# xtcyclist/hash_join_codes_KNL

Measured on AMD Instinct MI355X. Metric: probe Gtuples/s + % HBM roofline, PHJ |R|=64M join |S|=1G, 1/2/4/8 GPU, higher is better.
Workload: dtype u32

## Files before the change

### hash_join_codes_knl_amd/build.py

```python
import os
import shutil
import subprocess
import sys

PKG = os.path.dirname(os.path.abspath(__file__))
ROOT = os.path.dirname(PKG)
CSRC = os.path.join(PKG, "csrc")
HOST = os.path.join(PKG, "host")
LIB = os.path.join(PKG, "lib")
ARCH = "gfx950"

KERNEL_SOURCES = ["partition_kernels.hip", "join_kernels.hip", "npj_kernels.hip",
                  "gen_kernels.hip", "audit_kernels.hip", "hjgpu_api.hip", "hjgpu_ops.hip", "hjgpu_colops.hip", "hjgpu_host.hip", "hjgpu_multi.hip"]
HOST_PROGRAMS = {"npj": "npj_main.cpp", "phj": "phj_main.cpp", "cpra": "cpra_main.cpp",
                 "write": "write_main.cpp"}


def _hipcc():
    for cand in (os.environ.get("HIPCC"), shutil.which("hipcc"), "/opt/rocm/bin/hipcc"):
        if cand and os.path.exists(cand):
            return cand
    raise RuntimeError("hipcc not found (ROCm toolchain required to build libhjgpu)")


KERNEL_HASH_FILES = ["partition_kernels.hip", "join_kernels.hip", "npj_kernels.hip", "hj_device.hpp",
                     "hj_emit.hpp", "hj_lookup.hpp", "hj_internal.hpp", "scatter_layout.hpp", "hjgpu_ctx.hpp", "hjgpu_api.hip", "hjgpu_ops.hip",
                     "hjgpu_colops.hip", "colop_checks.hpp"]


def kernel_hash():
    import hashlib
    h = hashlib.sha256()
    for f in KERNEL_HASH_FILES:
        with open(os.path.join(CSRC, f), "rb") as fh:
            h.update(fh.read())
    return h.hexdigest()[:16]


def library_hash():
    import hashlib
    h = hashlib.sha256()
    for f in sorted(os.listdir(CSRC)):
        if f.endswith((".hip", ".hpp")):
            h.update(f.encode())
            with open(os.path.join(CSRC, f), "rb") as fh:
                h.update(fh.read())
    with open(os.path.join(ROOT, "include", "hjgpu.h"), "rb") as fh:
        h.update(fh.read())
    return h.hexdigest()[:16]


def _newer(target, deps):
    if not os.path.exists(target):
        return True
    t = os.path.getmtime(target)
    return any(os.path.getmtime(d) > t for d in deps if os.path.exists(d))


def lib_path():
# ... 65 lines not shown
```

### hash_join_codes_knl_amd/csrc/hjgpu_api.hip

```cpp
#include "hjgpu_ctx.hpp"
#include "hj_device.hpp"

using namespace hjapi;



namespace hjapi {


int fail(hjgpu_ctx *ctx, int status, const char *what, hipError_t e)
{
    if (ctx) {
        if (e != hipSuccess)
            snprintf(ctx->err, sizeof(ctx->err), "%s: %s", what, hipGetErrorString(e));
        else
            snprintf(ctx->err, sizeof(ctx->err), "%s", what);
    }
    return status;
}

static int release(hjgpu_ctx *ctx, void *p)
{
    if (!p) return HJGPU_OK;
    HIPCHK(ctx, hipFree(p));
// ... 189 lines not shown
    uint32_t f1 = prm ? prm->fanout1 : 0, f2 = prm ? prm->fanout2 : 0;
    *big_tables = false;
    if (f1 == 0) {
        double target = tune.join.cap() * 0.85;
        double parts = ceil((double)inner / target);
        if (parts > HJGPU_MAX_PARTS) {
            *big_tables = true;
            target = hj_join_config_big().cap() * 0.85;
            parts = ceil((double)inner / target);
        }
        if (parts < 64) parts = 64;
        if (parts > HJGPU_MAX_PARTS) parts = HJGPU_MAX_PARTS;
        if (parts <= 640) { f1 = (uint32_t)parts; f2 = 1; }
        else {
            f1 = 2;
            while ((double)f1 * f1 * 2.0 < parts) f1 <<= 1;
            if (f1 > 256) f1 = 256;
            if (parts >= 192.0 * 64.0) f1 = 192;
            f2 = (uint32_t)ceil(parts / f1);
            while (f2 > HJGPU_MAX_FANOUT) { f1 <<= 1; f2 = (uint32_t)ceil(parts / f1); }
            while ((u64)f1 * f2 > HJGPU_MAX_PARTS) --f2;
        }
    } else if (f2 == 0) f2 = 1;
    *F1 = f1; *F2 = f2;
}

void record(hjgpu_ctx *ctx, int which, hipStream_t s)
{
    if (ctx->ev_cur) {
        if (which == EV_BEGIN || which == EV_S_HIST || which == EV_S_PLAN || which == EV_S_SC1 || which == EV_S_SC2 || which == EV_JOIN)
            (void)hipEventRecord(ctx->ev_cur[which], s);
        return;
    }
    if (which == EV_BEGIN) { ctx->stats_override = false; ctx->grp_ev_groups = 0; ctx->last_lookup = false; }
    ctx->ev_valid[which] = (hipEventRecord(ctx->ev[which], s) == hipSuccess);
}

int audit_begin(hjgpu_ctx *ctx, int kind, size_t inner, size_t outer, hipStream_t stream, u64 **rec)
{
    *rec = nullptr;
    if (!ctx->tune.audit) return HJGPU_OK;
    const size_t words = (size_t)HJ_AUDIT_STAGES * 4;
    CHK(ensure(ctx, ctx->audit, (size_t)HJ_AUDIT_RING * words * sizeof(u64)));
    u64 *r = reinterpret_cast<u64 *>(ctx->audit.p) + (size_t)(ctx->audit_seq % HJ_AUDIT_RING) * words;
    HIPCHK(ctx, hj_zero_async(r, words * sizeof(u64), stream));
    CHK(hj_audit_meta(r + 4 * (HJ_AUDIT_STAGES - 1), ctx->audit_seq, (u64)kind, (u64)inner, (u64)outer, stream));
    ctx->audit_seq += 1;
    ctx->audit_checks.clear();
    *rec = r;
    return HJGPU_OK;
}

int audit_partitions(hjgpu_ctx *ctx, int stage, const u64 *tuples, const u64 *beg, const u64 *end, uint32_t parts, const HjAuditHash &h, u64 *rec,
                     hipStream_t stream)
{
    ctx->audit_checks.push_back(hjgpu_ctx::AuditCheck{stage, tuples, beg, end, parts, h});
    return hj_audit_partitions(tuples, beg, end, parts, h, rec + 4 * stage, ctx->cus, stream);
}

int refuse_capture(hjgpu_ctx *ctx, hipStream_t stream)
{
    hipStreamCaptureStatus status = hipStreamCaptureStatusNone;
    if (hipStreamIsCapturing(stream, &status) != hipSuccess) { (void)hipGetLastError(); return HJGPU_OK; }
    if (status != hipStreamCaptureStatusNone)
        return fail(ctx, HJGPU_EINVAL, "the stream is capturing a HIP graph: hjgpu joins cannot be captured");
    return HJGPU_OK;
}
// ... 283 lines not shown
    if (pl->F2 > 1 && pl->C == 1 && !ctx->tune.dense2 && ctx->tune.batch_tuples > 0 && pl->F1 <= 1024) {
        const u64 target = (u64)ctx->tune.batch_tuples;
        const u64 tile = gs.tile;
        const u64 tiles = hj_tiles_of(0, outer, 0, (uint32_t)tile) + 1;
        const u64 k = (tiles + ranges_of(ctx->tune, tiles, pl->F1) - 1) / ranges_of(ctx->tune, tiles, pl->F1) + 1;
        const u64 rpb = std::max<u64>(1, target / (k * tile));
        const u64 nb = (gs.ranges_per_chunk + rpb - 1) / rpb + 1;
        if (outer >= 3 * target) {
            pl->batch_ranges = (uint32_t)rpb; pl->batch_cap = (uint32_t)nb; pl->batch_tile_cap = (uint32_t)k;
            const u64 bound = rpb * k * tile;
            pl->tdesc_b_cap = (size_t)(bound / (u64)hj_scatter_tile(ctx->tune, 2, pl->F2, true) + 2 * (u64)pl->F1 + 8);
            pl->batch_bytes = (size_t)(bound + 64) * sizeof(u64);
            CHK(ensure(ctx, ctx->tmp[1], pl->batch_bytes));
            CHK(ensure(ctx, ctx->tmp[3], pl->batch_bytes));
        }
    }
    if (hj_mode_marks_build(pl->mode)) CHK(ensure(ctx, ctx->build_bits, build_bits_bytes(*pl, inner)));
    MetaLayout sz = carve(nullptr, pl->C, pl->F1, pl->P, pl->ranges, pl->items_extra, pl->tiles2, pl->batch_cap, pl->tdesc_b_cap);
    CHK(ensure(ctx, ctx->meta, sz.total_bytes));
    CHK(ensure(ctx, ctx->state, sizeof(DevState)));
    return HJGPU_OK;
}

namespace {

const int EV_OF_S[4] = {EV_S_HIST, EV_S_PLAN, EV_S_SC1, EV_S_SC2};
const int EV_OF_R[4] = {EV_R_HIST, EV_R_PLAN, EV_R_SC1, EV_R_SC2};

struct PhjRoad {
    bool pad2;
    bool merged;
    bool claim;
    bool joins;
};

PhjRoad phj_road(const hjgpu_ctx *ctx, const PhjPlan &pl, const Rel &R, const Rel &S, const EnqueueOpts &o)
{
    PhjRoad w;
    const bool audited = ctx->tune.audit && !o.grp;
    w.pad2 = pl.F2 > 1 && !ctx->tune.dense2;
    const bool resident = o.stages == PHJ_WHOLE && !o.inner_ready && !o.pre;
    w.merged = o.grp || (resident && !pl.batch_ranges && ctx->tune.merged_plan);
    w.claim = w.merged && !o.grp && pl.claim_s && !audited && pl.C == 1 && w.pad2;
    w.joins = R.rows && (S.rows || hj_mode_build_alone(pl.mode)) && o.stages != PHJ_BUILD_ONLY;
    return w;
}

struct PhjRun {
    hjgpu_ctx *ctx;
    const PhjPlan &pl;
    const EnqueueOpts &o;
    const PhjRoad road;
    hipStream_t stream;
    MetaLayout m;
    DevState *st;
    Pass1Geom geom[2];
    const uint32_t *in_k[2], *in_v[2];
    size_t nn[2];
    uint32_t *t1[4], *t2[4];
    PlanArgs pa;
    const u64 *dyn[2];
    u64 *audit = nullptr;
    bool p_major = false;
    uint32_t batches_used = 0;

    PhjRun(hjgpu_ctx *c, const PhjPlan &p, const Rel &R, const Rel &S, const EnqueueOpts &opts, hipStream_t s)
        : ctx(c), pl(p), o(opts), road(phj_road(c, p, R, S, opts)), stream(s),
          m(carve(c->meta.p, p.C, p.F1, p.P, p.ranges, p.items_extra, p.tiles2, p.batch_cap, p.tdesc_b_cap)),
          st(reinterpret_cast<DevState *>(c->state.p)),
          geom{make_geom(c->tune, R.keys, R.rows, p.C, p.F1, true), make_geom(c->tune, S.keys, S.rows, p.C, p.F1, true)},
          in_k{R.keys, S.keys}, in_v{R.vals, S.vals}, nn{R.rows, S.rows},
          t1{(uint32_t *)c->tmp[0].p, nullptr, (uint32_t *)c->tmp[2].p, nullptr},
          t2{(uint32_t *)c->tmp[4].p, nullptr, (uint32_t *)c->tmp[6].p, nullptr},
          dyn{opts.grp ? opts.grp->desc : nullptr, opts.grp ? opts.grp->desc + 2 : nullptr} {}

    bool pieces(int r) const { return o.pre && o.pre->tuples[r]; }

    int setup()
    {
        for (int r = 0; r < 2; ++r) {
            if (pieces(r)) geom[r].align = 0;
            if (!o.pre && (size_t)geom[r].ranges_per_chunk * pl.C > pl.ranges)
                return fail(ctx, HJGPU_EINVAL, "internal: the relation needs more pass-1 ranges than the plan's tables hold");
        }
        pa = plan_args(ctx, m, pl.C, pl.F1, pl.F2, (uint32_t)hj_scatter_tile(ctx->tune, 1, pl.F1, true),
                       (uint32_t)hj_scatter_tile(ctx->tune, 2, pl.F2, true), pl.unique, 0u);
        pa.cap = (uint32_t)hj_join_config_of(ctx->tune, pl.big_tables).cap();
        pa.tdesc_cap = (uint32_t)m.tdesc_cap;
        pa.multi_fill = m.tickets + HJ_TICKET_MULTI_FILL;
        pa.anti = hj_mode_keeps_unmatched(pl.mode) ? 1u : 0u;
        pa.pad2 = road.pad2 ? 1u : 0u;
        p_major = pl.C > 1 && road.pad2 && !o.pre;
        pa.p_major = p_major ? 1u : 0u;
        pa.seg_interleave = (o.pre && pl.C > 1 && road.pad2 && ctx->tune.piece_interleave) ? 1u : 0u;
        if (road.claim) pa.s_cap2 = pl.cap2;
        for (int r = 0; r < 2; ++r) {
            pa.tdesc[r] = m.tdesc[r]; pa.seg2[r] = m.seg2[r]; pa.more[r] = m.more[r]; pa.dyn[r] = dyn[r];
            pa.n[r] = pieces(r) ? o.pre->ch[r].b[pl.C] : nn[r];
            pa.regular[r] = pieces(r) ? 0u : 1u; pa.chunk_part[r] = geom[r].part;
            for (uint32_t c = 0; c < 9; ++c) pa.chunk_beg[r][c] = pieces(r) ? o.pre->ch[r].b[c <= pl.C ? c : pl.C] : geom[r].beg(c);
            pa.in_align[r] = o.pre ? 0u : align_of(in_k[r]);
        }
        return HJGPU_OK;
    }

    int begin()
    {
// ... 8 lines not shown
            HIPCHK(ctx, hj_zero_async(zt, (size_t)(ze - zt), stream));
        }
        if (o.stages == PHJ_PROBE_ONLY) HIPCHK(ctx, hj_zero_async(z1, (size_t)(ze - z1), stream));
        if (o.stages != PHJ_BUILD_ONLY && !o.grp) HIPCHK(ctx, hj_zero_async(st, sizeof(DevState), stream));
        return HJGPU_OK;
    }

    int audit_input(int r)
    {
        if (!audit || !nn[r]) return HJGPU_OK;
        u64 *rec = audit + 4 * (r ? 0 : 3);
        if (o.pre) return o.pre->tuples[r] ? hj_audit_sums_packed(o.pre->tuples[r], o.pre->ch[r].b[0], o.pre->ch[r].b[pl.C], rec, ctx->cus, stream) : HJGPU_OK;
        return in_k[r] ? hj_audit_sums_columns(in_k[r], in_v[r], nn[r], rec, ctx->cus, stream) : HJGPU_OK;
    }
    int audit_pass1(int r)
    {
        if (!audit || !nn[r] || o.pre || pl.C != 1 || pl.F2 <= 1) return HJGPU_OK;
        const HjAuditHash h = {pl.f1, pl.F1, 0u, 1u, 1u, pl.F1};
        return audit_partitions(ctx, r ? 1 : 4, reinterpret_cast<const u64 *>(ctx->tmp[2 * r].p), m.off1[r], nullptr, pl.F1, h, audit, stream);
    }
    int audit_final(int r)
    {
        if (!audit || !nn[r]) return HJGPU_OK;
        const bool two = pl.F2 > 1;
        const u64 *fin_r = reinterpret_cast<const u64 *>(two ? ctx->tmp[4 + 2 * r].p : ctx->tmp[2 * r].p);
        const HjAuditHash h = {o.pre ? pl.pre_f1 : pl.f1, o.pre ? pl.pre_F1tot : pl.F1, o.pre ? pl.pre_base : 0u, pl.f2, pl.F2, pl.P};
        return audit_partitions(ctx, r ? 2 : 5, fin_r, m.off2[r], m.end2[r], (road.pad2 ? 1u : pl.C) * pl.P, h, audit, stream);
    }

    int histogram(int r)
    {
        if (!nn[r]) return HJGPU_OK;
        return hj_launch_hist2(in_k[r], geom[r], pl.f1, pl.F1, pl.f2, pl.F2, m.counts[r],
                               m.range_counts[r], m.tickets + HJ_TICKET_K4 + HJ_MAX_CHUNKS * r, ctx->cus, stream, 0, dyn[r]);
    }
    int plan(uint32_t mask)
    {
        pa.mask = mask;
        return hj_launch_plan(pa, stream);
    }
    int range_bases(int r)
    {
        if (!nn[r]) return HJGPU_OK;
        return hj_launch_range_base(m.range_counts[r], m.off1[r], m.range_base[r], pl.C, geom[r].ranges_per_chunk, pl.F1, stream);
    }
    int pass1(int r)
    {
        if (!nn[r]) return HJGPU_OK;
        ScatterArgs sa = scatter_pass1(ctx, m, r, geom[r], pl.F1, pl.f1, in_k[r], in_v[r], t1[2 * r], t1[2 * r + 1]);
        sa.dyn = dyn[r];
        if (road.claim && r == 1) {
            sa.range_base = nullptr;
            sa.claim_cursors = m.claim1; sa.claim_cap = pl.cap1; sa.claim_overflow = &st->probe_overflow;
        }
        return hj_launch_scatter(sa, ctx->tune, scatter_cus(ctx), stream);
    }
    int pass2(int r, const uint32_t *in, int batch)
    {
        if (!nn[r] || pl.F2 <= 1) return HJGPU_OK;
        ScatterArgs sa = scatter_pass2(ctx, m, r, geom[r], pl, road.pad2, in, t2[2 * r]);
        if (p_major) { sa.seg_off = m.seg2[r]; sa.nseg = pl.F1; }
        if (batch >= 0) {
            const size_t b = (size_t)batch;
            sa.seg_off = m.boff + b * (pl.F1 + 1); sa.tile_prefix = m.tp2b + b * (pl.F1 + 1);
            sa.tile_desc = m.tdescb + b * pl.tdesc_b_cap * 2; sa.nseg = pl.F1; sa.work_counter = m.btickets + 2 * b + 1;
        }
        if (road.claim && r == 1) {
            sa.tile_prefix = m.claim_total; sa.nseg = 0; sa.seg_off = nullptr;
            sa.claim_overflow = &st->probe_overflow;
        }
        return hj_launch_scatter(sa, ctx->tune, scatter_cus(ctx), stream);
    }

    int partition_pieces(int r, uint32_t plan_mask, const int ev[4])
    {
        if (nn[r] && o.pre->counts[r])
            HIPCHK(ctx, hj_copy_async(m.counts[r], o.pre->counts[r], (size_t)pl.C * pl.P * sizeof(u64), stream));
        else if (nn[r]) CHK(hj_launch_hist_packed(o.pre->tuples[r], o.pre->ch[r], pl.pre_f1, pl.pre_F1tot, pl.pre_base, pl.F1,
                                                  pl.f2, pl.F2, m.counts[r], ctx->cus, stream));
        record(ctx, ev[0], stream);
        CHK(plan(plan_mask));
        record(ctx, ev[1], stream);
        record(ctx, ev[2], stream);
        CHK(pass2(r, reinterpret_cast<const uint32_t *>(o.pre->tuples[r]), -1));
        record(ctx, ev[3], stream);
        CHK(audit_input(r)); CHK(audit_final(r));
        return HJGPU_OK;
    }

    uint32_t probe_batches() const
    {
        const int r = 1;
        if (!pl.batch_ranges || !nn[r]) return 0;
        const u64 tiles = hj_tiles_of(0, nn[r], geom[r].align, geom[r].tile);
        const u64 k = (tiles + geom[r].ranges_per_chunk - 1) / geom[r].ranges_per_chunk;
        const u64 nb = (geom[r].ranges_per_chunk + pl.batch_ranges - 1) / pl.batch_ranges;
        return (k + 1 <= pl.batch_tile_cap && nb <= pl.batch_cap && nb >= 2) ? (uint32_t)nb : 0;
    }
    int partition_batched(uint32_t plan_mask, const int ev[4], uint32_t batches)
    {
        const int r = 1;
        CHK(histogram(r));
        record(ctx, ev[0], stream);
        CHK(plan(plan_mask));
// ... 48 lines not shown
        if (o.inner_ready) HIPCHK(ctx, hipStreamWaitEvent(stream, o.inner_ready, 0));
        record(ctx, EV_WAITED, stream);
        if (o.stages == PHJ_WHOLE) CHK(partition_relation(0, 1u | 4u, EV_OF_R));
        if (o.stages == PHJ_BUILD_ONLY) CHK(partition_relation(0, 1u, EV_OF_R));
        if (o.stages == PHJ_PROBE_ONLY) {
            record(ctx, EV_OF_R[0], stream);
            CHK(plan(4u));
            for (int i = 1; i < 4; ++i) record(ctx, EV_OF_R[i], stream);
            CHK(audit_final(0));
        }
        return HJGPU_OK;
    }

    int partition_merged()
    {
        CHK(histogram(0)); if (!road.claim) CHK(histogram(1));
        record(ctx, EV_S_HIST, stream);
        CHK(plan(7u));
        CHK(range_bases(0)); if (!road.claim) CHK(range_bases(1));
        record(ctx, EV_S_PLAN, stream);
        CHK(pass1(0)); CHK(pass1(1));
        if (road.claim && nn[1])
            CHK(hj_launch_claimed_desc(m.claim1, pl.cap1, pl.F1, pl.F2, pa.tile2, m.tdesc[1], (uint32_t)m.tdesc_cap, m.claim_total,
                                       &st->probe_overflow, stream));
        record(ctx, EV_S_SC1, stream);
        CHK(pass2(0, t1[0], -1)); CHK(pass2(1, t1[2], -1));
        record(ctx, EV_S_SC2, stream);
        record(ctx, EV_WAITED, stream);
        for (int e : EV_OF_R) record(ctx, e, stream);
        for (int r = 0; r < 2; ++r) { CHK(audit_input(r)); CHK(audit_pass1(r)); CHK(audit_final(r)); }
        return HJGPU_OK;
    }

    int join(u64 bs, u64 bl, uint32_t workers)
    {
        const bool marks = hj_mode_marks_build(pl.mode), build_rows = hj_mode_reports_build(pl.mode);
        uint32_t *const *fin = pl.F2 > 1 ? t2 : t1;
        JoinArgs ja{};
        ja.rk = fin[0]; ja.rv = fin[1]; ja.sk = fin[2]; ja.sv = fin[3];
        ja.roff = m.off2[0]; ja.soff = m.off2[1];
        ja.rend = m.end2[0]; ja.send = m.end2[1];
        if (road.claim) {
            CHK(hj_launch_claimed_pieces(m.off2[1], m.end2[1], m.cur2[1], pl.P, m.pieces, m.pieces + 2 * (size_t)pl.P, stream));
            ja.soff = m.pieces; ja.send = m.pieces + 2 * (size_t)pl.P; ja.s_pieces = 1;
        }
        ja.slice_prefix = m.slice_prefix; ja.slices = m.slices; ja.item_part = m.item_part;
        ja.P = pl.P; ja.chunks = road.pad2 ? 1u : pl.C;
        ja.f1 = pl.f1; ja.F1 = pl.F1; ja.f2 = pl.f2; ja.F2 = pl.F2;
        if (o.pre) { ja.f1 = pl.pre_f1; ja.F1 = pl.pre_F1tot; ja.p1_base = pl.pre_base; }
        ja.tf0 = pl.tf0; ja.tf1 = pl.tf1;
        ja.s_align = 0;
        ja.packed = 1;
        ja.big_tables = pl.big_tables ? 1u : 0u;
        ja.unique = pl.first_match ? 1u : 0u;
        ja.mode = pl.mode;
        ja.result = &st->result;
        ja.work_counter = reinterpret_cast<u64 *>(m.tickets + HJ_TICKET_JOIN);
        ja.work_counter2 = reinterpret_cast<u64 *>(m.tickets + HJ_TICKET_JOIN2);
        ja.work_counter3 = reinterpret_cast<u64 *>(m.tickets + HJ_TICKET_JOIN3);
        ja.multi_fill = m.tickets + HJ_TICKET_MULTI_FILL;
        ja.resume = o.grp ? 1u : 0u;
        join_output(ctx, ja, o.out, bs, bl, st);
        if (marks) {
            ja.build_bits = reinterpret_cast<uint32_t *>(ctx->build_bits.p);
            HIPCHK(ctx, hj_zero_async(ja.build_bits, build_bits_bytes(pl, nn[0]), stream));
            if ((!nn[1] || build_rows) && bs && !o.grp) HIPCHK(ctx, hj_fill_async(ctx->final_offsets.p, 0xFFFFFFFFu, (size_t)workers * sizeof(u64), stream));
        }
        if (nn[1]) CHK(hj_launch_join(ja, ctx->tune, ctx->cus, stream));
        if (build_rows) CHK(hj_launch_build_rows(ja, ctx->tune, ctx->cus, stream));
        else if (marks) CHK(hj_launch_build_unmatched(ja, ctx->tune, ctx->cus, stream));
        if (audit) CHK(hj_audit_copy(reinterpret_cast<const u64 *>(&st->result), audit + 4 * 6, 4, stream));
        return HJGPU_OK;
    }
};

}

int phj_enqueue(hjgpu_ctx *ctx, const PhjPlan &pl, const Rel &R, const Rel &S, hipStream_t stream, const EnqueueOpts &o)
{
    CHK(refuse_capture(ctx, stream));
    if (o.grp && (o.pre || o.stages != PHJ_WHOLE || o.inner_ready)) return fail(ctx, HJGPU_EINVAL, "internal: a device-planned group is a whole join on resident columns");
    if ((o.pre != nullptr) != (pl.pre != 0)) return fail(ctx, HJGPU_EINVAL, "internal: plan and relations disagree about pre-partitioning");
    PhjRun run(ctx, pl, R, S, o, stream);
    const uint32_t workers = (uint32_t)hj_join_workers(ctx->tune, ctx->cus, pl.big_tables);
    u64 bs = 0, bl = 0;
    CHK(setup_output(ctx, o.out, workers, &bs, &bl, pl.mode));

    CHK(run.setup());
    record(ctx, EV_BEGIN, stream);
    CHK(run.begin());
    CHK(run.road.merged ? run.partition_merged() : run.partition_in_turn());
    if (hj_mode_marks_build(pl.mode) && (o.pre || o.stages != PHJ_WHOLE)) return fail(ctx, HJGPU_EINVAL, "internal: a join that marks its build rows is a whole join");
    if (run.road.joins) CHK(run.join(bs, bl, workers));
    record(ctx, EV_JOIN, stream);
    if (bs && run.road.joins && !o.grp) CHK(close_gaps(ctx, o.out, workers, bs, run.st, stream, pl.mode));
    record(ctx, EV_GAPS, stream);
    ctx->stats.fanout1 = pl.F1; ctx->stats.fanout2 = pl.F2; ctx->stats.buckets = 0; ctx->stats.batches = run.batches_used;
    ctx->last_algo = ALGO_PHJ;
    return HJGPU_OK;
}

static int finish_from(hjgpu_ctx *ctx, const DevState &h, hjgpu_result *result, const hjgpu_output *out)
{
    if (result) *result = h.result;
    if (h.zero_key) return fail(ctx, HJGPU_EZEROKEY, "NPJ: a build key is 0, the empty-bucket sentinel");
    if (h.overflow) return fail(ctx, HJGPU_EOVERFLOW, "materialised output exceeded its capacity");
    if (out && out->d_keys && h.dense != h.result.count && (h.result.count != 0 || h.dense != 0))
        return fail(ctx, HJGPU_EHIP, "internal: dense length != match count after close_gaps");
    return HJGPU_OK;
}

static int read_state(hjgpu_ctx *ctx, DevState &h, hipStream_t stream)
{
    HIPCHK(ctx, hipMemcpyAsync(&h, ctx->state.p, sizeof(DevState), hipMemcpyDeviceToHost, stream));
    HIPCHK(ctx, hipStreamSynchronize(stream));
    return HJGPU_OK;
}

int finish_blocking(hjgpu_ctx *ctx, hjgpu_result *result, const hjgpu_output *out, hipStream_t stream)
{
    DevState h;
    CHK(read_state(ctx, h, stream));
    return finish_from(ctx, h, result, out);
}
// ... 139 lines not shown
{
    if (prm) CHK(refuse_join_mode(ctx, prm->flags, entry));
    CHK(check_columns(ctx, rk, rv, inner));
    CHK(check_lookup_columns(ctx, sk, outer, vals_out, match_bits));
    CHK(check_select_bits(ctx, select_bits, match_bits, outer));
    HIPCHK(ctx, hipSetDevice(ctx->device));
    size_t buckets; uint32_t factor;
    CHK(refuse_capture(ctx, stream));
    CHK(npj_prepare(ctx, inner, prm, &buckets, &factor));
    const bool line = !ctx->tune.npj_refhash;
    CHK(npj_build_enqueue(ctx, rk, rv, inner, buckets, factor, stream, line));
    return npj_lookup_enqueue(ctx, sk, outer, {reinterpret_cast<const u64 *>(ctx->table.p), buckets, factor, line}, vals_out, match_bits, stream, select_bits);
}

__global__ void accumulate_flags_kernel(const DevState *__restrict__ st, u64 *__restrict__ flags)
{
    if (threadIdx.x == 0) { if (st->zero_key) hj_store(&flags[0], flags[0] + 1); if (st->overflow) hj_store(&flags[1], flags[1] + 1); }
}

const hjgpu_output *take_async_output(hjgpu_ctx *ctx, const hjgpu_output *given)
{
    if (given) return given;
    if (!ctx->has_pending_out) return nullptr;
    ctx->has_pending_out = false;
    return &ctx->pending_out;
}

}

static int phj_grouped(hjgpu_ctx *ctx, uint32_t G, uint32_t chunks, const Rel &R, const Rel &S, const hjgpu_phj_params *prm, const hjgpu_output *out,
                       hipStream_t stream);
static void grouped_caps(const hjgpu_ctx *ctx, uint32_t G, size_t inner, size_t outer, size_t *cap_r, size_t *cap_s, size_t *plan_inner);

extern "C" {

const char *hjgpu_status_string(int s)
{
    switch (s) {
    case HJGPU_OK: return "ok";
    case HJGPU_EINVAL: return "invalid argument";
    case HJGPU_EALIGN: return "column not 16-byte aligned";
    case HJGPU_ENOMEM: return "out of device memory";
    case HJGPU_EHIP: return "HIP runtime error";
    case HJGPU_EZEROKEY: return "key 0 is reserved by NPJ";
    case HJGPU_EOVERFLOW: return "output capacity exceeded";
    case HJGPU_ENODEVICE: return "no GPU device";
    case HJGPU_ERCCL: return "RCCL / communicator error";
    case HJGPU_ERANGE: return "row number out of range";
    default: return "unknown status";
    }
}

#ifndef HJGPU_KERNEL_HASH
#define HJGPU_KERNEL_HASH "unknown"
#endif
const char *hjgpu_kernel_hash(void) { return HJGPU_KERNEL_HASH; }
#ifndef HJGPU_LIBRARY_HASH
#define HJGPU_LIBRARY_HASH "unknown"
#endif
const char *hjgpu_library_hash(void) { return HJGPU_LIBRARY_HASH; }

int hjgpu_device_count(int *count)
{
    if (!count) return HJGPU_EINVAL;
    *count = 0;
    if (hipGetDeviceCount(count) != hipSuccess) { *count = 0; (void)hipGetLastError(); return HJGPU_ENODEVICE; }
    return HJGPU_OK;
}

int hjgpu_create(int device, hjgpu_ctx **out)
{
    if (!out) return HJGPU_EINVAL;
    *out = nullptr;
    int n = 0;
    if (hipGetDeviceCount(&n) != hipSuccess || n <= 0) return HJGPU_ENODEVICE;
    if (device < 0) { if (hipGetDevice(&device) != hipSuccess) return HJGPU_ENODEVICE; }
    if (device >= n) return HJGPU_EINVAL;
    hjgpu_ctx *ctx = new hjgpu_ctx();
    ctx->err[0] = 0;
    ctx->device = device;
    memset(&ctx->stats, 0, sizeof(ctx->stats));
    if (hipSetDevice(device) != hipSuccess ||
        hipGetDeviceProperties(&ctx->prop, device) != hipSuccess) { delete ctx; return HJGPU_ENODEVICE; }
    ctx->cus = ctx->prop.multiProcessorCount;
    hj_tuning_from_env(&ctx->tune);
    for (int i = 0; i < EV_COUNT; ++i) {
        ctx->ev_valid[i] = false;
        if (hipEventCreate(&ctx->ev[i]) != hipSuccess) { delete ctx; return HJGPU_EHIP; }
    }
    *out = ctx;
    return HJGPU_OK;
}

int hjgpu_destroy(hjgpu_ctx *ctx)
{
    if (!ctx) return HJGPU_OK;
    (void)hipSetDevice(ctx->device);
    (void)hipDeviceSynchronize();
    DevBuf *all[] = {&ctx->tmp[0], &ctx->tmp[1], &ctx->tmp[2], &ctx->tmp[3], &ctx->tmp[4], &ctx->tmp[5],
                     &ctx->tmp[6], &ctx->tmp[7], &ctx->meta, &ctx->table, &ctx->state, &ctx->moves,
                     &ctx->final_offsets, &ctx->build_bits, &ctx->grp[0], &ctx->grp[1], &ctx->grp[2], &ctx->grp[3], &ctx->grp_off, &ctx->audit, &ctx->audit_lay, &ctx->compact, &ctx->group, &ctx->count_words};
    for (DevBuf *b : all) if (b->p) (void)hipFree(b->p);
    for (int i = 0; i < EV_COUNT; ++i) (void)hipEventDestroy(ctx->ev[i]);
    if (ctx->aux) (void)hipStreamDestroy(ctx->aux);
    for (hipEvent_t e : ctx->grp_ev) if (e) (void)hipEventDestroy(e);
    for (hipEvent_t e : ctx->grp_ev_pass0) if (e) (void)hipEventDestroy(e);
    for (int b = 0; b < 4; ++b) {
        if (ctx->host_stage[b]) (void)hipHostFree(ctx->host_stage[b]);
        if (ctx->host_stage_ev[b]) (void)hipEventDestroy(ctx->host_stage_ev[b]);
    }
    for (hipStream_t s : ctx->host_streams) if (s) (void)hipStreamDestroy(s);
    delete ctx;
    return HJGPU_OK;
}

const char *hjgpu_last_error(const hjgpu_ctx *ctx) { return ctx ? ctx->err : "null context"; }

int hjgpu_set_option(hjgpu_ctx *ctx, const char *name, const char *value)
{
    if (!ctx || !name || !value) return HJGPU_EINVAL;
    HjTuning t = ctx->tune;
    if (!hj_tuning_set(&t, name, value)) return fail(ctx, HJGPU_EINVAL, "hjgpu_set_option: unknown option or malformed value");
    if (!hj_join_config_built(t.join, false))
        return fail(ctx, HJGPU_EINVAL, "hjgpu_set_option: join_cfg names a geometry that is not built");
    if (t.unique && !hj_join_config_built(t.join, true))
        return fail(ctx, HJGPU_EINVAL, "hjgpu_set_option: this join_cfg geometry has no _UNIQUE instance (geometries with one: 512,13,2 and 1024,14,2)");
    ctx->tune = t;
    ctx->prepared = false;
    return HJGPU_OK;
}

int hjgpu_get_device_info(hjgpu_ctx *ctx, hjgpu_device_info *info)
{
    if (!ctx || !info) return HJGPU_EINVAL;
    memset(info, 0, sizeof(*info));
    snprintf(info->name, sizeof(info->name), "%s", ctx->prop.name);
    snprintf(info->arch, sizeof(info->arch), "%s", ctx->prop.gcnArchName);
    info->compute_units = ctx->cus;
    info->lds_bytes_per_block = (int)ctx->prop.sharedMemPerBlock;
    info->hbm_bytes = ctx->prop.totalGlobalMem;
    return HJGPU_OK;
}

int hjgpu_reserve(hjgpu_ctx *ctx, size_t inner, size_t outer)
{
    if (!ctx) return HJGPU_EINVAL;
    HIPCHK(ctx, hipSetDevice(ctx->device));
    PhjPlan pl;
    hjgpu_phj_params prm;
    memset(&prm, 0, sizeof(prm));
    const uint32_t groups = grouped_groups(ctx, inner, outer, nullptr);
    if (groups > 1 && outer) {
        ReserveClock clock(ctx);
        size_t cap_r, cap_s, plan_inner;
        grouped_caps(ctx, groups, inner, outer, &cap_r, &cap_s, &plan_inner);
        CHK(grouped_twins(ctx, group_layout(groups), inner, outer));
        CHK(phj_prepare(ctx, cap_r, cap_s, &prm, 8, &pl, {.plan_inner = plan_inner}));
    } else {
        CHK(phj_prepare(ctx, inner, outer, &prm, 8, &pl));
        if (claimed_probe_allowed(ctx)) CHK(phj_prepare(ctx, inner, outer, &prm, 1, &pl, {.claim_s = true}));
    }
    size_t buckets; uint32_t factor;
    CHK(npj_prepare(ctx, inner, nullptr, &buckets, &factor));
    return HJGPU_OK;
}

static size_t lds_lookup_rows(const HjTuning &tune);
int hjgpu_get_counter(hjgpu_ctx *ctx, const char *name, uint64_t *value)
{
    if (!ctx || !name || !value) return HJGPU_EINVAL;
    if (strcmp(name, "probe_fallbacks") == 0) { *value = ctx->probe_fallbacks; return HJGPU_OK; }
    if (strcmp(name, "probe_exact") == 0) { *value = (ctx->tune.exact_probe_counts || ctx->probe_exact) ? 1u : 0u; return HJGPU_OK; }
    if (strcmp(name, "lookup_lds_rows") == 0) { *value = lds_lookup_rows(ctx->tune); return HJGPU_OK; }
    if (strcmp(name, "compact_ranges") == 0) { *value = hj_compact::ranges_of(ctx->cus); return HJGPU_OK; }
    if (strcmp(name, "compact_chunk_rows") == 0) { *value = hj_compact::CHUNK_ROWS; return HJGPU_OK; }
    if (strcmp(name, "group_lds_groups") == 0) { *value = hj_group::LDS_GROUPS; return HJGPU_OK; }
    if (strcmp(name, "filter_step_rows") == 0) { *value = hj_filter::step_rows(ctx->cus); return HJGPU_OK; }
    if (strcmp(name, "gather_step_rows") == 0) { *value = hj_gather::step_rows(ctx->cus); return HJGPU_OK; }
    return fail(ctx, HJGPU_EINVAL, "unknown counter (probe_fallbacks, probe_exact, lookup_lds_rows, compact_ranges, compact_chunk_rows, group_lds_groups, filter_step_rows, gather_step_rows)");
}

static void fill_reserve(const hjgpu_ctx *ctx, hjgpu_stats *s)
{
    s->ms_reserve = ctx->ms_reserve;
    s->placement_tried = ctx->placement_tried; s->placement_timeboxed = ctx->placement_timeboxed;
    s->placement_fill_ms = ctx->placement_fill_ms; s->placement_search_ms = ctx->placement_search_ms; s->placement_bytes = (uint64_t)ctx->placement_bytes;
}

int hjgpu_get_stats(hjgpu_ctx *ctx, hjgpu_stats *s)
{
    if (!ctx || !s) return HJGPU_EINVAL;
    if (ctx->stats_override) {
        *s = ctx->stats;
        fill_reserve(ctx, s);
        return HJGPU_OK;
    }
    if (ctx->grp_ev_groups) {
        HIPCHK(ctx, hipEventSynchronize(ctx->grp_ev_pass0[2]));
        auto between = [&](hipEvent_t a, hipEvent_t b) -> float { float ms = 0; return hipEventElapsedTime(&ms, a, b) == hipSuccess ? ms : 0.f; };
        hjgpu_stats r = ctx->stats;
        r.ms_histogram = r.ms_plan = r.ms_scatter1 = r.ms_scatter2 = r.ms_join = r.ms_close_gaps = r.ms_build = r.ms_inner_wait = 0;
        for (uint32_t g = 0; g < ctx->grp_ev_groups; ++g) {
            const hipEvent_t *e = ctx->grp_ev.data() + (size_t)g * EV_COUNT;
            r.ms_histogram += between(e[EV_BEGIN], e[EV_S_HIST]);
            r.ms_plan += between(e[EV_S_HIST], e[EV_S_PLAN]);
            r.ms_scatter1 += between(e[EV_S_PLAN], e[EV_S_SC1]);
            r.ms_scatter2 += between(e[EV_S_SC1], e[EV_S_SC2]);
            r.ms_join += between(e[EV_S_SC2], e[EV_JOIN]);
        }
        r.ms_scatter0 = between(ctx->grp_ev_pass0[0], ctx->grp_ev_pass0[1]);
        r.ms_total = between(ctx->grp_ev_pass0[0], ctx->grp_ev_pass0[2]);
        r.ms_close_gaps = r.ms_total - (r.ms_scatter0 + r.ms_histogram + r.ms_plan + r.ms_scatter1 + r.ms_scatter2 + r.ms_join);
        if (r.ms_close_gaps < 0) r.ms_close_gaps = 0;
        r.groups = ctx->grp_ev_groups;
        fill_reserve(ctx, &r);
        *s = r;
        return HJGPU_OK;
    }
    if (ctx->ev_valid[EV_GAPS]) HIPCHK(ctx, hipEventSynchronize(ctx->ev[EV_GAPS]));
    auto span = [&](int a, int b) -> float {
        float ms = 0;
        if (ctx->ev_valid[a] && ctx->ev_valid[b] &&
            hipEventElapsedTime(&ms, ctx->ev[a], ctx->ev[b]) == hipSuccess) return ms;
        return 0.f;
    };
    hjgpu_stats r = ctx->stats;
    r.ms_total = span(EV_BEGIN, EV_GAPS);
    r.ms_inner_wait = 0;
    fill_reserve(ctx, &r);
    if (ctx->last_algo >= ALGO_ONE_KERNEL) {
        memset(&r, 0, sizeof(r));
        r.ms_total = span(EV_BEGIN, EV_GAPS);
        r.ms_histogram = span(EV_BEGIN, EV_S_HIST);
        r.ms_join = span(EV_S_HIST, EV_JOIN);
        if (ctx->last_algo == ALGO_GROUP_SUM) r.ms_close_gaps = span(EV_JOIN, EV_GAPS);
        fill_reserve(ctx, &r);
        *s = r;
        return HJGPU_OK;
    }
    if (ctx->last_algo == ALGO_NPJ) {
        r.ms_build = span(EV_BEGIN, EV_R_HIST);
        r.ms_join = span(EV_R_HIST, EV_JOIN);
        r.ms_histogram = r.ms_plan = r.ms_scatter1 = r.ms_scatter2 = 0;
    } else {
        r.ms_histogram = span(EV_BEGIN, EV_S_HIST) + span(EV_WAITED, EV_R_HIST);
        r.ms_plan = span(EV_S_HIST, EV_S_PLAN) + span(EV_R_HIST, EV_R_PLAN);
        r.ms_scatter1 = span(EV_S_PLAN, EV_S_SC1) + span(EV_R_PLAN, EV_R_SC1);
        r.ms_scatter2 = span(EV_S_SC1, EV_S_SC2) + span(EV_R_SC1, EV_R_SC2);
        r.ms_inner_wait = span(EV_S_SC2, EV_WAITED);
        r.ms_join = span(EV_R_SC2, EV_JOIN);
        r.ms_build = 0;
    }
    r.ms_close_gaps = ctx->last_lookup ? 0.f : span(EV_JOIN, EV_GAPS);
    r.ms_scatter0 = 0; r.groups = 0;
    *s = r;
    return HJGPU_OK;
}

int hjgpu_get_async_status(hjgpu_ctx *ctx, void *stream_)
{
    if (!ctx) return HJGPU_EINVAL;
    if (!ctx->state.p) return HJGPU_OK;
    hipStream_t stream = (hipStream_t)stream_;
    HIPCHK(ctx, hipSetDevice(ctx->device));
    DevState h;
    CHK(read_state(ctx, h, stream));
    if (ctx->grp_last.valid && h.group_skew) {
        const hjgpu_ctx::GroupedCall c = ctx->grp_last;
        ctx->grp_last.valid = false;
        const hjgpu_phj_params *prm = c.has_prm ? &c.prm : nullptr;
        const hjgpu_output *out = c.has_out ? &c.out : nullptr;
        const uint32_t groups = grouped_groups(ctx, c.R.rows, c.S.rows, prm);
        if (groups > 1) CHK(phj_grouped(ctx, groups, c.chunks, c.R, c.S, prm, out, stream));
        else {
            PhjPlan pl;
            CHK(phj_prepare(ctx, c.R.rows, c.S.rows, prm, c.chunks, &pl));
// ... 698 lines not shown
```

### hash_join_codes_knl_amd/csrc/hjgpu_ctx.hpp

```cpp
#pragma once
#include <hip/hip_runtime.h>
#include <algorithm>
#include <chrono>
#include <functional>
#include <math.h>
#include <stdio.h>
#include <stdlib.h>
#include <string.h>
#include <thread>
#include <vector>

#include "hj_internal.hpp"
#include "colop_checks.hpp"


struct DevBuf {
    void *p = nullptr;
    size_t cap = 0;
};

namespace hjapi {
struct Rel { const uint32_t *keys = nullptr, *vals = nullptr; size_t rows = 0; };
}

struct DevState {
    hjgpu_result result;
    u64 block_counter;
    u64 dense;
    u64 work_counter;
    uint32_t overflow;
    uint32_t zero_key;
    uint32_t nmoves;
    uint32_t pad;
    u64 work_counter2;
    uint32_t group_skew;
    uint32_t probe_overflow;
};

enum { EV_BEGIN = 0, EV_S_HIST, EV_S_PLAN, EV_S_SC1, EV_S_SC2, EV_WAITED,
       EV_R_HIST, EV_R_PLAN, EV_R_SC1, EV_R_SC2, EV_JOIN, EV_GAPS, EV_COUNT };

enum Algo { ALGO_NONE = -1, ALGO_NPJ = 0, ALGO_PHJ = 1,
            ALGO_ONE_KERNEL = 2,
            ALGO_COMPACT = 3, ALGO_GROUP_SUM = 4, ALGO_FILTER = 5, ALGO_GATHER = 6 };

struct hjgpu_ctx {
    int device = 0;
    int cus = 0;
    hipDeviceProp_t prop;
    char err[512];
    DevBuf tmp[8];
    DevBuf meta;
    DevBuf table;
    DevBuf state;
    DevBuf moves;
    DevBuf final_offsets;
    DevBuf compact;
    DevBuf group;
    DevBuf count_words;
    DevBuf build_bits;
    hipEvent_t ev[EV_COUNT];
    bool ev_valid[EV_COUNT];
    hjgpu_stats stats;
    Algo last_algo = ALGO_NONE;
    bool last_lookup = false;
    bool prepared = false;
    size_t prepared_inner = 0, prepared_max_outer = 0;
    unsigned char prepared_plan[128];
    HjTuning tune;
    hipStream_t host_streams[3] = {nullptr, nullptr, nullptr};
    void *host_stage[4] = {nullptr, nullptr, nullptr, nullptr};
    hipEvent_t host_stage_ev[4] = {nullptr, nullptr, nullptr, nullptr};
    hjgpu_output pending_out;
    bool has_pending_out = false;
    bool last_had_output = false;
    uint64_t probe_fallbacks = 0;
    bool probe_exact = false;
    bool rows_plain = false;
    DevBuf grp[4], grp_off;
    bool stats_override = false;
    hipStream_t aux = nullptr;
    hipEvent_t *ev_cur = nullptr;
    std::vector<hipEvent_t> grp_ev;
    uint32_t grp_ev_groups = 0;
    hipEvent_t grp_ev_pass0[3] = {nullptr, nullptr, nullptr};
    struct GroupedCall {
        bool valid = false;
        uint32_t chunks = 1;
        hjapi::Rel R, S;
        bool has_prm = false, has_out = false;
        hjgpu_phj_params prm;
        hjgpu_output out;
        hjgpu_result *d_result = nullptr;
    } grp_last;
    DevBuf audit, audit_lay;
    uint64_t audit_seq = 0;
    struct AuditCheck { int stage; const u64 *tuples, *beg, *end; uint32_t parts; HjAuditHash h; };
    std::vector<AuditCheck> audit_checks;
    float ms_reserve = 0;
    uint32_t placement_tried = 0, placement_timeboxed = 0;
    float placement_fill_ms = 0, placement_search_ms = 0;
    size_t placement_bytes = 0;
};

namespace hjapi {

const uint32_t DEFAULT_F1 = 0x9E3779B1u, DEFAULT_F2 = 0x85EBCA6Bu;
const uint32_t DEFAULT_TF0 = 0xC2B2AE35u, DEFAULT_TF1 = 0x27D4EB2Fu;
const uint32_t DEFAULT_NPJ_FACTOR = 0x9E3779B1u;
const uint32_t DEFAULT_F0 = 0x7FEB352Du;
// ... 181 lines not shown
```

Baseline: 126.9.

## Partition build side on a side stream concurrently with probe scatter pass

Adds a 'build beside' path that forks a second stream and runs the build relation's histogram, plan, range bases and both scatter passes on a small CU budget, while the probe relation's first scatter pass runs on the main stream with the remaining CUs. The probe's second pass waits only on the plan event, and the streams rejoin before the join. The aim is to hide build-side partitioning behind the much larger probe-side scatter instead of running the two in turn. The cost is contention for HBM bandwidth and a smaller CU count for each pass. It is enabled by default when claim-mode merged planning applies and the probe side is at least 12 times the build side.

```diff
diff --git a/hash_join_codes_knl_amd/build.py b/hash_join_codes_knl_amd/build.py
--- a/hash_join_codes_knl_amd/build.py
+++ b/hash_join_codes_knl_amd/build.py
@@ -24,7 +24,7 @@
 
 
 KERNEL_HASH_FILES = ["partition_kernels.hip", "join_kernels.hip", "npj_kernels.hip", "hj_device.hpp",
-                     "hj_emit.hpp", "hj_lookup.hpp", "hj_internal.hpp", "scatter_layout.hpp", "hjgpu_ctx.hpp", "hjgpu_api.hip", "hjgpu_ops.hip",
+                     "hj_emit.hpp", "hj_lookup.hpp", "hj_internal.hpp", "scatter_layout.hpp", "build_beside_layout.hpp", "hjgpu_ctx.hpp", "hjgpu_api.hip", "hjgpu_ops.hip",
                      "hjgpu_colops.hip", "colop_checks.hpp"]
 
 
diff --git a/hash_join_codes_knl_amd/csrc/build_beside_layout.hpp b/hash_join_codes_knl_amd/csrc/build_beside_layout.hpp
--- /dev/null
+++ b/hash_join_codes_knl_amd/csrc/build_beside_layout.hpp
@@ -0,0 +1,27 @@
+#pragma once
+#include <stddef.h>
+#include <stdint.h>
+
+namespace hj_beside {
+constexpr int DEFAULT_BUILD_CUS = 32;
+constexpr int MIN_CUS = 128;
+constexpr uint64_t MIN_PROBE_ROWS = 1u << 20;
+constexpr uint64_t MIN_PROBE_PER_BUILD = 12;
+
+struct Split {
+    int build, probe;
+    constexpr bool overlap() const { return build > 0; }
+};
+
+constexpr Split split(int cus, int build_cus, uint64_t inner_rows, uint64_t outer_rows)
+{
+    const Split none = {0, cus};
+    if (cus < 2 || inner_rows == 0 || outer_rows == 0 || build_cus < 0) return none;
+    if (build_cus == 0) {
+        if (DEFAULT_BUILD_CUS == 0 || cus < MIN_CUS || outer_rows < MIN_PROBE_ROWS || outer_rows / MIN_PROBE_PER_BUILD < inner_rows) return none;
+        build_cus = DEFAULT_BUILD_CUS;
+    }
+    const int b = build_cus < cus - 1 ? build_cus : cus - 1;
+    return Split{b, cus - b};
+}
+}
diff --git a/hash_join_codes_knl_amd/csrc/hjgpu_api.hip b/hash_join_codes_knl_amd/csrc/hjgpu_api.hip
--- a/hash_join_codes_knl_amd/csrc/hjgpu_api.hip
+++ b/hash_join_codes_knl_amd/csrc/hjgpu_api.hip
@@ -245,7 +245,7 @@
             (void)hipEventRecord(ctx->ev_cur[which], s);
         return;
     }
-    if (which == EV_BEGIN) { ctx->stats_override = false; ctx->grp_ev_groups = 0; ctx->last_lookup = false; }
+    if (which == EV_BEGIN) { ctx->stats_override = false; ctx->grp_ev_groups = 0; ctx->last_lookup = false; ctx->last_beside = false; }
     ctx->ev_valid[which] = (hipEventRecord(ctx->ev[which], s) == hipSuccess);
 }
 
@@ -595,6 +595,8 @@
     bool merged;
     bool claim;
     bool joins;
+    bool beside;
+    hj_beside::Split split;
 };
 
 PhjRoad phj_road(const hjgpu_ctx *ctx, const PhjPlan &pl, const Rel &R, const Rel &S, const EnqueueOpts &o)
@@ -606,6 +608,9 @@
     w.merged = o.grp || (resident && !pl.batch_ranges && ctx->tune.merged_plan);
     w.claim = w.merged && !o.grp && pl.claim_s && !audited && pl.C == 1 && w.pad2;
     w.joins = R.rows && (S.rows || hj_mode_build_alone(pl.mode)) && o.stages != PHJ_BUILD_ONLY;
+    w.split = hj_beside::split(scatter_cus(ctx), ctx->build_cus, R.rows, S.rows);
+    w.beside = w.claim && w.joins && ctx->build_beside && !ctx->rows_plain && w.split.overlap();
+    if (!w.beside) w.split = hj_beside::Split{0, scatter_cus(ctx)};
     return w;
 }
 
@@ -626,6 +631,8 @@
     u64 *audit = nullptr;
     bool p_major = false;
     uint32_t batches_used = 0;
+    hipStream_t on[2];
+    int hist_cus[2], k6_cus[2];
 
     PhjRun(hjgpu_ctx *c, const PhjPlan &p, const Rel &R, const Rel &S, const EnqueueOpts &opts, hipStream_t s)
         : ctx(c), pl(p), o(opts), road(phj_road(c, p, R, S, opts)), stream(s),
@@ -635,7 +642,8 @@
           in_k{R.keys, S.keys}, in_v{R.vals, S.vals}, nn{R.rows, S.rows},
           t1{(uint32_t *)c->tmp[0].p, nullptr, (uint32_t *)c->tmp[2].p, nullptr},
           t2{(uint32_t *)c->tmp[4].p, nullptr, (uint32_t *)c->tmp[6].p, nullptr},
-          dyn{opts.grp ? opts.grp->desc : nullptr, opts.grp ? opts.grp->desc + 2 : nullptr} {}
+          dyn{opts.grp ? opts.grp->desc : nullptr, opts.grp ? opts.grp->desc + 2 : nullptr},
+          on{s, s}, hist_cus{c->cus, c->cus}, k6_cus{scatter_cus(c), scatter_cus(c)} {}
 
     bool pieces(int r) const { return o.pre && o.pre->tuples[r]; }
 
@@ -710,17 +718,18 @@
     {
         if (!nn[r]) return HJGPU_OK;
         return hj_launch_hist2(in_k[r], geom[r], pl.f1, pl.F1, pl.f2, pl.F2, m.counts[r],
-                               m.range_counts[r], m.tickets + HJ_TICKET_K4 + HJ_MAX_CHUNKS * r, ctx->cus, stream, 0, dyn[r]);
-    }
-    int plan(uint32_t mask)
+                               m.range_counts[r], m.tickets + HJ_TICKET_K4 + HJ_MAX_CHUNKS * r, hist_cus[r], on[r], 0, dyn[r]);
+    }
+    int plan(uint32_t mask) { return plan(mask, stream); }
+    int plan(uint32_t mask, hipStream_t s)
     {
         pa.mask = mask;
-        return hj_launch_plan(pa, stream);
+        return hj_launch_plan(pa, s);
     }
     int range_bases(int r)
     {
         if (!nn[r]) return HJGPU_OK;
-        return hj_launch_range_base(m.range_counts[r], m.off1[r], m.range_base[r], pl.C, geom[r].ranges_per_chunk, pl.F1, stream);
+        return hj_launch_range_base(m.range_counts[r], m.off1[r], m.range_base[r], pl.C, geom[r].ranges_per_chunk, pl.F1, on[r]);
     }
     int pass1(int r)
     {
@@ -731,7 +740,7 @@
             sa.range_base = nullptr;
             sa.claim_cursors = m.claim1; sa.claim_cap = pl.cap1; sa.claim_overflow = &st->probe_overflow;
         }
-        return hj_launch_scatter(sa, ctx->tune, scatter_cus(ctx), stream);
+        return hj_launch_scatter(sa, ctx->tune, k6_cus[r], on[r]);
     }
     int pass2(int r, const uint32_t *in, int batch)
     {
@@ -747,7 +756,7 @@
             sa.tile_prefix = m.claim_total; sa.nseg = 0; sa.seg_off = nullptr;
             sa.claim_overflow = &st->probe_overflow;
         }
-        return hj_launch_scatter(sa, ctx->tune, scatter_cus(ctx), stream);
+        return hj_launch_scatter(sa, ctx->tune, k6_cus[r], on[r]);
     }
 
     int partition_pieces(int r, uint32_t plan_mask, const int ev[4])
@@ -862,6 +871,53 @@
         return HJGPU_OK;
     }
 
+    int partition_beside()
+    {
+        if (!ctx->side) HIPCHK(ctx, hipStreamCreateWithFlags(&ctx->side, hipStreamNonBlocking));
+        for (hipEvent_t &e : ctx->beside_ev) if (!e) HIPCHK(ctx, hipEventCreate(&e));
+        hipEvent_t *ev = ctx->beside_ev;
+        const hipStream_t side = ctx->side;
+        on[0] = side; hist_cus[0] = k6_cus[0] = road.split.build; k6_cus[1] = road.split.probe;
+        HIPCHK(ctx, hipEventRecord(ev[hjgpu_ctx::BESIDE_FORK], stream));
+        HIPCHK(ctx, hipStreamWaitEvent(side, ev[hjgpu_ctx::BESIDE_FORK], 0));
+        struct Joined {
+            hipEvent_t done; hipStream_t side, main; bool armed = true;
+            hipError_t now()
+            {
+                armed = false;
+                hipError_t e = hipEventRecord(done, side);
+                if (e == hipSuccess) e = hipStreamWaitEvent(main, done, 0);
+                if (e != hipSuccess) (void)hipStreamSynchronize(side);
+                return e;
+            }
+            ~Joined() { if (armed) (void)now(); }
+        } joined{ev[hjgpu_ctx::BESIDE_R_DONE], side, stream};
+        record(ctx, EV_S_HIST, stream);
+        record(ctx, EV_S_PLAN, stream);
+        CHK(pass1(1));
+        CHK(histogram(0));
+        record(ctx, EV_R_HIST, side);
+        CHK(plan(7u, side));
+        HIPCHK(ctx, hipEventRecord(ev[hjgpu_ctx::BESIDE_PLAN_DONE], side));
+        CHK(range_bases(0));
+        record(ctx, EV_R_PLAN, side);
+        CHK(pass1(0));
+        record(ctx, EV_R_SC1, side);
+        CHK(pass2(0, t1[0], -1));
+        record(ctx, EV_R_SC2, side);
+        CHK(hj_launch_claimed_desc(m.claim1, pl.cap1, pl.F1, pl.F2, pa.tile2, m.tdesc[1], (uint32_t)m.tdesc_cap, m.claim_total,
+                                   &st->probe_overflow, stream));
+        record(ctx, EV_S_SC1, stream);
+        HIPCHK(ctx, hipStreamWaitEvent(stream, ev[hjgpu_ctx::BESIDE_PLAN_DONE], 0));
+        CHK(pass2(1, t1[2], -1));
+        record(ctx, EV_S_SC2, stream);
+        HIPCHK(ctx, joined.now());
+        record(ctx, EV_WAITED, stream);
+        ctx->last_beside = true;
+        ++ctx->beside_joins;
+        return HJGPU_OK;
+    }
+
     int join(u64 bs, u64 bl, uint32_t workers)
     {
         const bool marks = hj_mode_marks_build(pl.mode), build_rows = hj_mode_reports_build(pl.mode);
@@ -919,7 +975,7 @@
     CHK(run.setup());
     record(ctx, EV_BEGIN, stream);
     CHK(run.begin());
-    CHK(run.road.merged ? run.partition_merged() : run.partition_in_turn());
+    CHK(run.road.beside ? run.partition_beside() : run.road.merged ? run.partition_merged() : run.partition_in_turn());
     if (hj_mode_marks_build(pl.mode) && (o.pre || o.stages != PHJ_WHOLE)) return fail(ctx, HJGPU_EINVAL, "internal: a join that marks its build rows is a whole join");
     if (run.road.joins) CHK(run.join(bs, bl, workers));
     record(ctx, EV_JOIN, stream);
@@ -1125,6 +1181,25 @@
                        hipStream_t stream);
 static void grouped_caps(const hjgpu_ctx *ctx, uint32_t G, size_t inner, size_t outer, size_t *cap_r, size_t *cap_s, size_t *plan_inner);
 
+static bool beside_option(hjgpu_ctx *ctx, const char *name, const char *value, bool *ok)
+{
+    const bool flag = strcmp(name, "build_beside") == 0;
+    if (!flag && strcmp(name, "build_cus") != 0) return false;
+    char *end = nullptr;
+    const long x = strtol(value, &end, 10);
+    *ok = end != value && !*end && x >= 0 && (flag || x < ctx->cus || x == 0);
+    if (*ok && flag) ctx->build_beside = x != 0;
+    if (*ok && !flag) ctx->build_cus = (int)x;
+    return true;
+}
+
+static void beside_option_from_env(hjgpu_ctx *ctx, const char *name, const char *env)
+{
+    const char *v = getenv(env);
+    bool ok = true;
+    if (v && *v && beside_option(ctx, name, v, &ok) && !ok) fprintf(stderr, "hjgpu: ignoring malformed %s=%s\n", env, v);
+}
+
 extern "C" {
 
 const char *hjgpu_status_string(int s)
@@ -1177,6 +1252,8 @@
         hipGetDeviceProperties(&ctx->prop, device) != hipSuccess) { delete ctx; return HJGPU_ENODEVICE; }
     ctx->cus = ctx->prop.multiProcessorCount;
     hj_tuning_from_env(&ctx->tune);
+    beside_option_from_env(ctx, "build_beside", "HJGPU_BUILD_BESIDE");
+    beside_option_from_env(ctx, "build_cus", "HJGPU_BUILD_CUS");
     for (int i = 0; i < EV_COUNT; ++i) {
         ctx->ev_valid[i] = false;
         if (hipEventCreate(&ctx->ev[i]) != hipSuccess) { delete ctx; return HJGPU_EHIP; }
@@ -1196,6 +1273,8 @@
     for (DevBuf *b : all) if (b->p) (void)hipFree(b->p);
     for (int i = 0; i < EV_COUNT; ++i) (void)hipEventDestroy(ctx->ev[i]);
     if (ctx->aux) (void)hipStreamDestroy(ctx->aux);
+    for (hipEvent_t e : ctx->beside_ev) if (e) (void)hipEventDestroy(e);
+    if (ctx->side) (void)hipStreamDestroy(ctx->side);
     for (hipEvent_t e : ctx->grp_ev) if (e) (void)hipEventDestroy(e);
     for (hipEvent_t e : ctx->grp_ev_pass0) if (e) (void)hipEventDestroy(e);
     for (int b = 0; b < 4; ++b) {
@@ -1212,6 +1291,9 @@
 int hjgpu_set_option(hjgpu_ctx *ctx, const char *name, const char *value)
 {
     if (!ctx || !name || !value) return HJGPU_EINVAL;
+    bool ok = false;
+    if (beside_option(ctx, name, value, &ok))
+        return ok ? HJGPU_OK : fail(ctx, HJGPU_EINVAL, "hjgpu_set_option: build_beside is 0 or 1, build_cus 0 (the library's choice) or 1 ... CUs - 1");
     HjTuning t = ctx->tune;
     if (!hj_tuning_set(&t, name, value)) return fail(ctx, HJGPU_EINVAL, "hjgpu_set_option: unknown option or malformed value");
     if (!hj_join_config_built(t.join, false))
@@ -1263,6 +1345,7 @@
 {
     if (!ctx || !name || !value) return HJGPU_EINVAL;
     if (strcmp(name, "probe_fallbacks") == 0) { *value = ctx->probe_fallbacks; return HJGPU_OK; }
+    if (strcmp(name, "build_beside") == 0) { *value = ctx->beside_joins; return HJGPU_OK; }
     if (strcmp(name, "probe_exact") == 0) { *value = (ctx->tune.exact_probe_counts || ctx->probe_exact) ? 1u : 0u; return HJGPU_OK; }
     if (strcmp(name, "lookup_lds_rows") == 0) { *value = lds_lookup_rows(ctx->tune); return HJGPU_OK; }
     if (strcmp(name, "compact_ranges") == 0) { *value = hj_compact::ranges_of(ctx->cus); return HJGPU_OK; }
@@ -1270,7 +1353,7 @@
     if (strcmp(name, "group_lds_groups") == 0) { *value = hj_group::LDS_GROUPS; return HJGPU_OK; }
     if (strcmp(name, "filter_step_rows") == 0) { *value = hj_filter::step_rows(ctx->cus); return HJGPU_OK; }
     if (strcmp(name, "gather_step_rows") == 0) { *value = hj_gather::step_rows(ctx->cus); return HJGPU_OK; }
-    return fail(ctx, HJGPU_EINVAL, "unknown counter (probe_fallbacks, probe_exact, lookup_lds_rows, compact_ranges, compact_chunk_rows, group_lds_groups, filter_step_rows, gather_step_rows)");
+    return fail(ctx, HJGPU_EINVAL, "unknown counter (probe_fallbacks, probe_exact, build_beside, lookup_lds_rows, compact_ranges, compact_chunk_rows, group_lds_groups, filter_step_rows, gather_step_rows)");
 }
 
 static void fill_reserve(const hjgpu_ctx *ctx, hjgpu_stats *s)
@@ -1335,6 +1418,15 @@
         r.ms_build = span(EV_BEGIN, EV_R_HIST);
         r.ms_join = span(EV_R_HIST, EV_JOIN);
         r.ms_histogram = r.ms_plan = r.ms_scatter1 = r.ms_scatter2 = 0;
+    } else if (ctx->last_beside) {
+        float ms = 0;
+        r.ms_histogram = (ctx->ev_valid[EV_R_HIST] && hipEventElapsedTime(&ms, ctx->beside_ev[hjgpu_ctx::BESIDE_FORK], ctx->ev[EV_R_HIST]) == hipSuccess) ? ms : 0.f;
+        r.ms_plan = span(EV_R_HIST, EV_R_PLAN);
+        r.ms_scatter1 = span(EV_S_PLAN, EV_S_SC1);
+        r.ms_scatter2 = span(EV_S_SC1, EV_S_SC2);
+        r.ms_inner_wait = span(EV_S_SC2, EV_WAITED);
+        r.ms_join = span(EV_WAITED, EV_JOIN);
+        r.ms_build = 0;
     } else {
         r.ms_histogram = span(EV_BEGIN, EV_S_HIST) + span(EV_WAITED, EV_R_HIST);
         r.ms_plan = span(EV_S_HIST, EV_S_PLAN) + span(EV_R_HIST, EV_R_PLAN);
diff --git a/hash_join_codes_knl_amd/csrc/hjgpu_ctx.hpp b/hash_join_codes_knl_amd/csrc/hjgpu_ctx.hpp
--- a/hash_join_codes_knl_amd/csrc/hjgpu_ctx.hpp
+++ b/hash_join_codes_knl_amd/csrc/hjgpu_ctx.hpp
@@ -12,6 +12,7 @@
 
 #include "hj_internal.hpp"
 #include "colop_checks.hpp"
+#include "build_beside_layout.hpp"
 
 
 struct DevBuf {
@@ -76,6 +77,13 @@
     bool last_had_output = false;
     uint64_t probe_fallbacks = 0;
     bool probe_exact = false;
+    enum { BESIDE_FORK = 0, BESIDE_PLAN_DONE, BESIDE_R_DONE, BESIDE_EVENTS };
+    hipStream_t side = nullptr;
+    hipEvent_t beside_ev[BESIDE_EVENTS] = {nullptr, nullptr, nullptr};
+    bool build_beside = true;
+    int build_cus = 0;
+    uint64_t beside_joins = 0;
+    bool last_beside = false;
     bool rows_plain = false;
     DevBuf grp[4], grp_off;
     bool stats_override = false;
```

Measured after the change: 131.9 (median of 6 runs). 1.04x the previous value.
